# lukashermann/hulc

Hardware: AMD Instinct MI355X
Metric: trajectory-windows/sec (seq_len=32, bs=64/GPU) (higher is better)
Workload: dtype bf16; 1 GPU; HULC training step, vision goal only (use_clip_auxiliary_loss=false), B=64 windows/GPU, seq_len=32, 200x200 static + 84x84 gripper fp32 NCHW frames, fwd+loss+bwd+Adam, dropout 0.1; global_batch=64, seq_len=32, parallelism=dp1

## Files before the change

### hulc_amd/csrc/common.h

```cpp
#pragma once
#include <hip/hip_runtime.h>
#include <stdint.h>

void hulc_set_error(const char* fmt, ...);

#define HIP_CHECK(x)                                                                                     \
    do {                                                                                                 \
        hipError_t e_ = (x);                                                                             \
        if (e_ != hipSuccess) {                                                                          \
            hulc_set_error("%s:%d: %s -> %s", __FILE__, __LINE__, #x, hipGetErrorString(e_));            \
            return 1;                                                                                    \
        }                                                                                                \
    } while (0)

#define DEVI __device__ __forceinline__

#if defined(__HIP_DEVICE_COMPILE__) || defined(__HIPCC__)
__device__ __forceinline__ void lds_dma16(const void* src, unsigned lds_addr) {
    const unsigned a = (unsigned)__builtin_amdgcn_readfirstlane((int)lds_addr);
    asm volatile("s_mov_b32 m0, %1\n\ts_nop 0\n\tglobal_load_lds_dwordx4 %0, off" : : "v"(src), "s"(a) : "memory", "m0");
}
#endif


#ifdef HULC_HALF_F16
#define HULC_NS hulc_f16
#define HULC_HALF_NAME "fp16"
#else
#define HULC_NS hulc_bf16
#define HULC_HALF_NAME "bf16"
#endif

namespace HULC_NS {

typedef uint16_t h16_t;
typedef float f32x4 __attribute__((ext_vector_type(4)));
typedef float f32x2_t __attribute__((ext_vector_type(2)));

#ifdef HULC_HALF_F16
typedef _Float16 h16x8_t __attribute__((ext_vector_type(8)));
typedef _Float16 h16x2_t __attribute__((ext_vector_type(2)));
#define MFMA_16x16x32_H __builtin_amdgcn_mfma_f32_16x16x32_f16
DEVI float h2f(h16_t x) { return (float)*reinterpret_cast<const _Float16*>(&x); }
DEVI h16_t f2h(float f) {
    _Float16 b = (_Float16)f;
    return *reinterpret_cast<h16_t*>(&b);
}
#else
typedef __bf16 h16x8_t __attribute__((ext_vector_type(8)));
typedef __bf16 h16x2_t __attribute__((ext_vector_type(2)));
#define MFMA_16x16x32_H __builtin_amdgcn_mfma_f32_16x16x32_bf16
DEVI float h2f(h16_t x) { return __uint_as_float(((uint32_t)x) << 16); }
DEVI h16_t f2h(float f) {
    __bf16 b = (__bf16)f;
    return *reinterpret_cast<h16_t*>(&b);
}
#endif
DEVI unsigned pack2h(float lo, float hi) {
    h16x2_t b = __builtin_convertvector(f32x2_t{lo, hi}, h16x2_t);
    return *reinterpret_cast<unsigned*>(&b);
}
DEVI float h2f_lo(unsigned w) { return h2f((h16_t)(w & 0xffffu)); }
DEVI float h2f_hi(unsigned w) {
#ifdef HULC_HALF_F16
    return h2f((h16_t)(w >> 16));
#else
    return __uint_as_float(w & 0xffff0000u);
#endif
}
template <typename T> DEVI float to_f(T x);
template <> DEVI float to_f<float>(float x) { return x; }
template <> DEVI float to_f<h16_t>(h16_t x) { return h2f(x); }
template <typename T> DEVI T from_f(float x);
template <> DEVI float from_f<float>(float x) { return x; }
template <> DEVI h16_t from_f<h16_t>(float x) { return f2h(x); }

template <typename T> struct Vec8 { T v[8]; };

template <typename T> DEVI void load8(const T* p, T (&v)[8]);
template <> DEVI void load8<h16_t>(const h16_t* p, h16_t (&v)[8]) {
    if ((((uintptr_t)p) & 15) == 0) {
        uint4 u = *reinterpret_cast<const uint4*>(p);
        *reinterpret_cast<uint4*>(v) = u;
    } else {
#pragma unroll
        for (int i = 0; i < 8; ++i) v[i] = p[i];
    }
}
template <> DEVI void load8<float>(const float* p, float (&v)[8]) {
    if ((((uintptr_t)p) & 15) == 0) {
        float4 a = reinterpret_cast<const float4*>(p)[0];
        float4 b = reinterpret_cast<const float4*>(p)[1];
        v[0] = a.x; v[1] = a.y; v[2] = a.z; v[3] = a.w; v[4] = b.x; v[5] = b.y; v[6] = b.z; v[7] = b.w;
    } else {
#pragma unroll
        for (int i = 0; i < 8; ++i) v[i] = p[i];
    }
}
template <typename T> DEVI void load8_guard(const T* p, int nvalid, T (&v)[8]) {
    if (nvalid >= 8) { load8<T>(p, v); return; }
#pragma unroll
    for (int i = 0; i < 8; ++i) v[i] = (i < nvalid) ? p[i] : from_f<T>(0.f);
}
template <typename T> DEVI void zero8(T (&v)[8]) {
#pragma unroll
    for (int i = 0; i < 8; ++i) v[i] = from_f<T>(0.f);
}

DEVI float wave_sum(float x) {
#pragma unroll
    for (int o = 32; o > 0; o >>= 1) x += __shfl_xor(x, o, 64);
    return x;
}
DEVI float wave_max(float x) {
#pragma unroll
    for (int o = 32; o > 0; o >>= 1) x = fmaxf(x, __shfl_xor(x, o, 64));
    return x;
}

DEVI uint32_t hash_u32(uint64_t seed, uint64_t idx) {
    uint64_t z = seed + (idx + 1) * 0x9E3779B97F4A7C15ull;
    z = (z ^ (z >> 30)) * 0xBF58476D1CE4E5B9ull;
    z = (z ^ (z >> 27)) * 0x94D049BB133111EBull;
    z = z ^ (z >> 31);
    return (uint32_t)(z >> 32);
}
DEVI float hash_uniform(uint64_t seed, uint64_t idx) {
    return ((hash_u32(seed, idx) >> 8) + 0.5f) * (1.0f / 16777216.0f);
}

}
```

### hulc_amd/csrc/tr_fused.h

```cpp
#pragma once
#include "common.h"
#include "conv_wgrad.h"

namespace HULC_NS {

struct TrLayerP {
    const float* xin;
    int ln_in;
    const float *ln_g, *ln_b;
    float* xf_out; h16_t* xt_out; float* st_out;
    const h16_t *Wqkv, *Wo, *W1, *W2;
    const float *bqkv, *bo, *b1, *b2, *n1g, *n1b;
    h16_t* qkv; float* Pat; h16_t* ao; float* y1; float* st1; h16_t* x1t; float* x1f; h16_t* hff; float* y2;
    int B, S;
    float dp;
    unsigned long long seed_att, seed_o, seed_h, seed_y;
    long long* stamps;
};
#ifdef TRF_STAMPS
#define TRF_STAMP(i) do { if (p.stamps && blockIdx.x == 5 && tid == 0) p.stamps[i] = clock64(); } while (0)
#else
#define TRF_STAMP(i) do { } while (0)
#endif

constexpr int TRF_D = 128, TRF_FF = 2048, TRF_NH = 8, TRF_HD = 16, TRF_NQ = 4, TRF_HQ = TRF_FF / TRF_NQ;
constexpr int TRF_XP = TRF_D * 2 + 32;
constexpr int TRF_HP = TRF_HQ * 2 + 32;
constexpr int TRF_QP = 3 * TRF_D * 2 + 16;
constexpr size_t TRF_LDS = 32 * TRF_D * 4 * 2 + 32 * TRF_XP * 3 + 32 * TRF_QP + 32 * TRF_HP;
constexpr size_t TRF_LDS_WIDE = TRF_LDS + 32 * TRF_QP;

template <bool WIDE>
__global__ void __launch_bounds__(512) tr_layer_fwd_kernel(TrLayerP p) {
    extern __shared__ __attribute__((aligned(16))) char smem[];
    typedef __attribute__((address_space(3))) float lds_f32;
    typedef __attribute__((address_space(3))) h16_t lds_h16;
    typedef unsigned int u32x2_t __attribute__((ext_vector_type(2)));
    lds_char* const xf = (lds_char*)smem;
    lds_char* const x1f = xf + 32 * TRF_D * 4;
    lds_char* const xb = x1f + 32 * TRF_D * 4;
    lds_char* const aob = xb + 32 * TRF_XP;
    lds_char* const x1b = aob + 32 * TRF_XP;
    lds_char* const qb = x1b + 32 * TRF_XP;
    lds_char* const hb = qb + (WIDE ? 64 : 32) * TRF_QP;
    const int tid = threadIdx.x, lane = tid & 63, wave = tid >> 6;
    const int li = lane & 15, g = lane >> 4;
    const int hq = blockIdx.x % TRF_NQ;
    const int w = WIDE ? blockIdx.x / (2 * TRF_NQ) : blockIdx.x / TRF_NQ, half = WIDE ? (blockIdx.x / TRF_NQ) & 1 : 0;
    const int SW = p.S;
    const int r0 = half * 32;
    const int S = WIDE ? min(32, SW - r0) : SW;
    const long long row0 = (long long)w * SW + r0;
    const bool lead = hq == 0;
    const bool mt1 = S > 16;
    const float keep = 1.f / (1.f - p.dp);

    TRF_STAMP(0);
    h16x8_t wq[3][4];
#pragma unroll
    for (int nt = 0; nt < 3; ++nt)
#pragma unroll
        for (int ks = 0; ks < 4; ++ks) wq[nt][ks] = *reinterpret_cast<const h16x8_t*>(wfrag_ptr(p.Wqkv, (3 * wave + nt) * 16, TRF_D, 0, lane) + ks * 512);

    f32x4 pbq[3], pb1[4];
#pragma unroll
    for (int nt = 0; nt < 3; ++nt) pbq[nt] = *reinterpret_cast<const f32x4*>(p.bqkv + (3 * wave + nt) * 16 + g * 4);
    const f32x4 pbo = *reinterpret_cast<const f32x4*>(p.bo + wave * 16 + g * 4);
    f32x4 pb2 = f32x4{0.f, 0.f, 0.f, 0.f};
    if (lead) pb2 = *reinterpret_cast<const f32x4*>(p.b2 + wave * 16 + g * 4);
    const float pn1g0 = p.n1g[lane], pn1g1 = p.n1g[lane + 64], pn1b0 = p.n1b[lane], pn1b1 = p.n1b[lane + 64];
    float plg0 = 0.f, plg1 = 0.f, plb0 = 0.f, plb1 = 0.f;
    if (p.ln_in) { plg0 = p.ln_g[lane]; plg1 = p.ln_g[lane + 64]; plb0 = p.ln_b[lane]; plb1 = p.ln_b[lane + 64]; }

    {
#pragma unroll
        for (int rr = 0; rr < 4; ++rr) {
            const int r = wave * 4 + rr;
            float v0 = 0.f, v1 = 0.f;
            if (r < S) {
                const float* xr = p.xin + (row0 + r) * TRF_D;
                v0 = xr[lane]; v1 = xr[lane + 64];
                if (p.ln_in) {
                    const float mean = wave_sum(v0 + v1) * (1.f / TRF_D);
                    const float d0 = v0 - mean, d1 = v1 - mean;
                    const float rstd = rsqrtf(wave_sum(d0 * d0 + d1 * d1) * (1.f / TRF_D) + 1e-5f);
                    v0 = d0 * rstd * plg0 + plb0;
                    v1 = d1 * rstd * plg1 + plb1;
                    if (lead) {
                        p.xf_out[(row0 + r) * TRF_D + lane] = v0; p.xf_out[(row0 + r) * TRF_D + lane + 64] = v1;
                        p.xt_out[(row0 + r) * TRF_D + lane] = f2h(v0); p.xt_out[(row0 + r) * TRF_D + lane + 64] = f2h(v1);
                        if (lane == 0) { p.st_out[2 * (row0 + r)] = mean; p.st_out[2 * (row0 + r) + 1] = rstd; }
                    }
                }
            }
            *(lds_f32*)(xf + (r * TRF_D + lane) * 4) = v0; *(lds_f32*)(xf + (r * TRF_D + lane + 64) * 4) = v1;
            *(lds_h16*)(xb + r * TRF_XP + lane * 2) = f2h(v0); *(lds_h16*)(xb + r * TRF_XP + (lane + 64) * 2) = f2h(v1);
        }
        if (WIDE) {
            const int o0 = 32 - r0, So = min(32, SW - o0);
            const long long orow0 = (long long)w * SW + o0;
#pragma unroll
            for (int rr = 0; rr < 4; ++rr) {
                const int r = wave * 4 + rr;
                float v0 = 0.f, v1 = 0.f;
                if (r < So) {
                    const float* xr = p.xin + (orow0 + r) * TRF_D;
                    v0 = xr[lane]; v1 = xr[lane + 64];
                    if (p.ln_in) {
                        const float mean = wave_sum(v0 + v1) * (1.f / TRF_D);
                        const float d0 = v0 - mean, d1 = v1 - mean;
                        const float rstd = rsqrtf(wave_sum(d0 * d0 + d1 * d1) * (1.f / TRF_D) + 1e-5f);
                        v0 = d0 * rstd * plg0 + plb0;
                        v1 = d1 * rstd * plg1 + plb1;
                    }
                }
                *(lds_h16*)(aob + r * TRF_XP + lane * 2) = f2h(v0); *(lds_h16*)(aob + r * TRF_XP + (lane + 64) * 2) = f2h(v1);
            }
        }
    }
    __syncthreads();
    h16x8_t wo[4], w1[4][4], w2[16];
#pragma unroll
    for (int ks = 0; ks < 4; ++ks) wo[ks] = *reinterpret_cast<const h16x8_t*>(wfrag_ptr(p.Wo, wave * 16, TRF_D, 0, lane) + ks * 512);

    TRF_STAMP(1);
    {
        f32x4 acc[3][2];
#pragma unroll
        for (int nt = 0; nt < 3; ++nt) { acc[nt][0] = f32x4{0.f, 0.f, 0.f, 0.f}; acc[nt][1] = f32x4{0.f, 0.f, 0.f, 0.f}; }
#pragma unroll
        for (int ks = 0; ks < 4; ++ks) {
            const h16x8_t b0 = *(__attribute__((address_space(3))) h16x8_t*)(xb + li * TRF_XP + ks * 64 + g * 16);
            const h16x8_t b1 = *(__attribute__((address_space(3))) h16x8_t*)(xb + (16 + li) * TRF_XP + ks * 64 + g * 16);
#pragma unroll
            for (int nt = 0; nt < 3; ++nt) {
                acc[nt][0] = MFMA_16x16x32_H(wq[nt][ks], b0, acc[nt][0], 0, 0, 0);
                if (mt1) acc[nt][1] = MFMA_16x16x32_H(wq[nt][ks], b1, acc[nt][1], 0, 0, 0);
            }
        }
#pragma unroll
        for (int nt = 0; nt < 3; ++nt) {
            const int n = (3 * wave + nt) * 16 + g * 4;
            const f32x4 bb = pbq[nt];
#pragma unroll
            for (int mt = 0; mt < 2; ++mt) {
                const int m = mt * 16 + li;
                u32x2_t o;
                o[0] = pack2h(acc[nt][mt][0] + bb[0], acc[nt][mt][1] + bb[1]);
                o[1] = pack2h(acc[nt][mt][2] + bb[2], acc[nt][mt][3] + bb[3]);
                *(__attribute__((address_space(3))) u32x2_t*)(qb + (r0 + m) * TRF_QP + n * 2) = o;
                if (lead && m < S) *reinterpret_cast<u32x2_t*>(p.qkv + (row0 + m) * (3 * TRF_D) + n) = o;
            }
        }
        if (WIDE) {
            const int o0 = 32 - r0;
#pragma unroll
            for (int nt = 0; nt < 3; ++nt) { acc[nt][0] = f32x4{0.f, 0.f, 0.f, 0.f}; acc[nt][1] = f32x4{0.f, 0.f, 0.f, 0.f}; }
#pragma unroll
            for (int ks = 0; ks < 4; ++ks) {
                const h16x8_t b0 = *(__attribute__((address_space(3))) h16x8_t*)(aob + li * TRF_XP + ks * 64 + g * 16);
                const h16x8_t b1 = *(__attribute__((address_space(3))) h16x8_t*)(aob + (16 + li) * TRF_XP + ks * 64 + g * 16);
#pragma unroll
                for (int nt = 0; nt < 3; ++nt) {
                    acc[nt][0] = MFMA_16x16x32_H(wq[nt][ks], b0, acc[nt][0], 0, 0, 0);
                    acc[nt][1] = MFMA_16x16x32_H(wq[nt][ks], b1, acc[nt][1], 0, 0, 0);
                }
            }
#pragma unroll
            for (int nt = 0; nt < 3; ++nt) {
                const int n = (3 * wave + nt) * 16 + g * 4;
                const f32x4 bb = pbq[nt];
#pragma unroll
                for (int mt = 0; mt < 2; ++mt) {
                    u32x2_t o;
                    o[0] = pack2h(acc[nt][mt][0] + bb[0], acc[nt][mt][1] + bb[1]);
                    o[1] = pack2h(acc[nt][mt][2] + bb[2], acc[nt][mt][3] + bb[3]);
                    *(__attribute__((address_space(3))) u32x2_t*)(qb + (o0 + mt * 16 + li) * TRF_QP + n * 2) = o;
                }
            }
        }
    }
#pragma unroll
    for (int nt = 0; nt < 4; ++nt) pb1[nt] = *reinterpret_cast<const f32x4*>(p.b1 + hq * TRF_HQ + wave * 64 + nt * 16 + g * 4);
    auto load_w1 = [&]() {
#pragma unroll
        for (int nt = 0; nt < 4; ++nt)
#pragma unroll
            for (int ks = 0; ks < 4; ++ks)
                w1[nt][ks] = *reinterpret_cast<const h16x8_t*>(wfrag_ptr(p.W1, hq * TRF_HQ + wave * 64 + nt * 16, TRF_D, 0, lane) + ks * 512);
    };
    if (!WIDE) load_w1();
    __syncthreads();

    TRF_STAMP(2);
    {
        const int h = wave, i = lane & 31, hf = lane >> 5;
        auto row16 = [&](const lds_char* r, float (&o)[TRF_HD]) {
            const u32x4_t a = *(const lds_u32x4*)r, b = *(const lds_u32x4*)(r + 16);
#pragma unroll
            for (int e = 0; e < 4; ++e) { o[2 * e] = h2f_lo(a[e]); o[2 * e + 1] = h2f_hi(a[e]); o[8 + 2 * e] = h2f_lo(b[e]); o[9 + 2 * e] = h2f_hi(b[e]); }
        };
        constexpr int HJ = WIDE ? 32 : 16;
        if (i < S) {
            float q[TRF_HD];
            row16(qb + (r0 + i) * TRF_QP + h * TRF_HD * 2, q);
#pragma unroll
            for (int d = 0; d < TRF_HD; ++d) q[d] *= 0.25f;
            float sc[HJ];
            float m = -INFINITY;
#pragma unroll
            for (int jj = 0; jj < HJ; ++jj) {
                const int j = hf * HJ + jj;
                float kk[TRF_HD];
                row16(qb + (j < SW ? j : 0) * TRF_QP + (TRF_D + h * TRF_HD) * 2, kk);
                float s = 0.f;
#pragma unroll
                for (int d = 0; d < TRF_HD; ++d) s += q[d] * kk[d];
                sc[jj] = j < SW ? s : -INFINITY;
                m = fmaxf(m, sc[jj]);
            }
            m = fmaxf(m, __shfl_xor(m, 32));
            float den = 0.f;
#pragma unroll
            for (int jj = 0; jj < HJ; ++jj) { sc[jj] = (hf * HJ + jj) < SW ? __expf(sc[jj] - m) : 0.f; den += sc[jj]; }
            den += __shfl_xor(den, 32);
            const float inv = 1.f / den;
            float o[TRF_HD];
#pragma unroll
            for (int d = 0; d < TRF_HD; ++d) o[d] = 0.f;
            const long long pbase = (((long long)w * TRF_NH + h) * SW + r0 + i) * SW;
#pragma unroll
            for (int jj = 0; jj < HJ; ++jj) {
                const int j = hf * HJ + jj;
                if (j < SW) {
                    float pr = sc[jj] * inv;
                    if (lead) p.Pat[pbase + j] = pr;
                    if (p.dp > 0.f) pr = hash_uniform(p.seed_att, (unsigned long long)(pbase + j)) < p.dp ? 0.f : pr * keep;
                    float vv[TRF_HD];
                    row16(qb + j * TRF_QP + (2 * TRF_D + h * TRF_HD) * 2, vv);
#pragma unroll
                    for (int d = 0; d < TRF_HD; ++d) o[d] += pr * vv[d];
                }
            }
#pragma unroll
            for (int d = 0; d < TRF_HD; ++d) o[d] += __shfl_xor(o[d], 32);
            u32x4_t ov;
#pragma unroll
            for (int e = 0; e < 4; ++e) ov[e] = hf ? pack2h(o[8 + 2 * e], o[9 + 2 * e]) : pack2h(o[2 * e], o[2 * e + 1]);
            *(lds_u32x4*)(aob + i * TRF_XP + (h * TRF_HD + hf * 8) * 2) = ov;
            if (lead) *reinterpret_cast<u32x4_t*>(p.ao + (row0 + i) * TRF_D + h * TRF_HD + hf * 8) = ov;
        } else {
            *(lds_u32x4*)(aob + i * TRF_XP + (h * TRF_HD + hf * 8) * 2) = u32x4_t{0u, 0u, 0u, 0u};
        }
    }
    __syncthreads();

    if (WIDE) load_w1();
#pragma unroll
    for (int ks = 0; ks < 16; ++ks) w2[ks] = *reinterpret_cast<const h16x8_t*>(wfrag_ptr(p.W2, wave * 16, TRF_FF, hq * TRF_HQ, lane) + ks * 512);
    TRF_STAMP(3);
    {
        f32x4 acc[2] = {f32x4{0.f, 0.f, 0.f, 0.f}, f32x4{0.f, 0.f, 0.f, 0.f}};
#pragma unroll
        for (int ks = 0; ks < 4; ++ks) {
            const h16x8_t b0 = *(__attribute__((address_space(3))) h16x8_t*)(aob + li * TRF_XP + ks * 64 + g * 16);
            acc[0] = MFMA_16x16x32_H(wo[ks], b0, acc[0], 0, 0, 0);
            if (mt1) {
                const h16x8_t b1 = *(__attribute__((address_space(3))) h16x8_t*)(aob + (16 + li) * TRF_XP + ks * 64 + g * 16);
                acc[1] = MFMA_16x16x32_H(wo[ks], b1, acc[1], 0, 0, 0);
            }
        }
        const int n = wave * 16 + g * 4;
        const f32x4 bb = pbo;
#pragma unroll
        for (int mt = 0; mt < 2; ++mt) {
            const int m = mt * 16 + li;
            lds_char* xr = xf + (m * TRF_D + n) * 4;
            const f32x4 res = *(__attribute__((address_space(3))) f32x4*)xr;
            f32x4 y;
#pragma unroll
            for (int r = 0; r < 4; ++r) {
                float v = acc[mt][r] + bb[r];
                if (p.dp > 0.f) v = hash_uniform(p.seed_o, (unsigned long long)((row0 + m) * TRF_D + n + r)) < p.dp ? 0.f : v * keep;
                y[r] = m < S ? v + res[r] : 0.f;
            }
            *(__attribute__((address_space(3))) f32x4*)xr = y;
            if (lead && m < S) *reinterpret_cast<f32x4*>(p.y1 + (row0 + m) * TRF_D + n) = y;
        }
    }
    __syncthreads();

    TRF_STAMP(4);
    {
#pragma unroll
        for (int rr = 0; rr < 4; ++rr) {
            const int r = wave * 4 + rr;
            float v0 = *(lds_f32*)(xf + (r * TRF_D + lane) * 4), v1 = *(lds_f32*)(xf + (r * TRF_D + lane + 64) * 4);
            float o0 = 0.f, o1 = 0.f;
            if (r < S) {
                const float mean = wave_sum(v0 + v1) * (1.f / TRF_D);
                const float d0 = v0 - mean, d1 = v1 - mean;
                const float rstd = rsqrtf(wave_sum(d0 * d0 + d1 * d1) * (1.f / TRF_D) + 1e-5f);
                o0 = d0 * rstd * pn1g0 + pn1b0;
                o1 = d1 * rstd * pn1g1 + pn1b1;
                if (lead) {
                    p.x1f[(row0 + r) * TRF_D + lane] = o0; p.x1f[(row0 + r) * TRF_D + lane + 64] = o1;
                    p.x1t[(row0 + r) * TRF_D + lane] = f2h(o0); p.x1t[(row0 + r) * TRF_D + lane + 64] = f2h(o1);
                    if (lane == 0) { p.st1[2 * (row0 + r)] = mean; p.st1[2 * (row0 + r) + 1] = rstd; }
                }
            }
            *(lds_f32*)(x1f + (r * TRF_D + lane) * 4) = o0; *(lds_f32*)(x1f + (r * TRF_D + lane + 64) * 4) = o1;
            *(lds_h16*)(x1b + r * TRF_XP + lane * 2) = f2h(o0); *(lds_h16*)(x1b + r * TRF_XP + (lane + 64) * 2) = f2h(o1);
        }
    }
    __syncthreads();

    TRF_STAMP(5);
    {
        f32x4 acc[4][2];
#pragma unroll
        for (int nt = 0; nt < 4; ++nt) { acc[nt][0] = f32x4{0.f, 0.f, 0.f, 0.f}; acc[nt][1] = f32x4{0.f, 0.f, 0.f, 0.f}; }
#pragma unroll
        for (int ks = 0; ks < 4; ++ks) {
            const h16x8_t b0 = *(__attribute__((address_space(3))) h16x8_t*)(x1b + li * TRF_XP + ks * 64 + g * 16);
            const h16x8_t b1 = *(__attribute__((address_space(3))) h16x8_t*)(x1b + (16 + li) * TRF_XP + ks * 64 + g * 16);
#pragma unroll
            for (int nt = 0; nt < 4; ++nt) {
                acc[nt][0] = MFMA_16x16x32_H(w1[nt][ks], b0, acc[nt][0], 0, 0, 0);
                if (mt1) acc[nt][1] = MFMA_16x16x32_H(w1[nt][ks], b1, acc[nt][1], 0, 0, 0);
            }
        }
#pragma unroll
        for (int nt = 0; nt < 4; ++nt) {
            const int nl = wave * 64 + nt * 16 + g * 4, n = hq * TRF_HQ + nl;
            const f32x4 bb = pb1[nt];
#pragma unroll
            for (int mt = 0; mt < 2; ++mt) {
                const int m = mt * 16 + li;
                float v[4];
#pragma unroll
                for (int r = 0; r < 4; ++r) {
                    v[r] = fmaxf(acc[nt][mt][r] + bb[r], 0.f);
                    if (p.dp > 0.f) v[r] = hash_uniform(p.seed_h, (unsigned long long)((row0 + m) * TRF_FF + n + r)) < p.dp ? 0.f : v[r] * keep;
                    if (m >= S) v[r] = 0.f;
                }
                u32x2_t o;
                o[0] = pack2h(v[0], v[1]); o[1] = pack2h(v[2], v[3]);
                *(__attribute__((address_space(3))) u32x2_t*)(hb + m * TRF_HP + nl * 2) = o;
                if (m < S) *reinterpret_cast<u32x2_t*>(p.hff + (row0 + m) * TRF_FF + n) = o;
            }
        }
    }
    __syncthreads();

    TRF_STAMP(6);
    {
        f32x4 acc[2] = {f32x4{0.f, 0.f, 0.f, 0.f}, f32x4{0.f, 0.f, 0.f, 0.f}};
#pragma unroll
        for (int ks = 0; ks < 16; ++ks) {
            const h16x8_t b0 = *(__attribute__((address_space(3))) h16x8_t*)(hb + li * TRF_HP + ks * 64 + g * 16);
            acc[0] = MFMA_16x16x32_H(w2[ks], b0, acc[0], 0, 0, 0);
            if (mt1) {
                const h16x8_t b1 = *(__attribute__((address_space(3))) h16x8_t*)(hb + (16 + li) * TRF_HP + ks * 64 + g * 16);
                acc[1] = MFMA_16x16x32_H(w2[ks], b1, acc[1], 0, 0, 0);
            }
        }
        const int n = wave * 16 + g * 4;
        const f32x4 bb = pb2;
#pragma unroll
        for (int mt = 0; mt < 2; ++mt) {
            const int m = mt * 16 + li;
            if (m >= S) continue;
            const f32x4 res = *(__attribute__((address_space(3))) f32x4*)(x1f + (m * TRF_D + n) * 4);
#pragma unroll
            for (int r = 0; r < 4; ++r) {
                float v = acc[mt][r] + bb[r];
                if (p.dp > 0.f) v = hash_uniform(p.seed_y, (unsigned long long)((row0 + m) * TRF_D + n + r)) < p.dp ? 0.f : v * keep;
                if (lead) v += res[r];
                unsafeAtomicAdd(p.y2 + (row0 + m) * TRF_D + n + r, v);
            }
        }
    }
    TRF_STAMP(7);
}

struct TrFfnBwdP {
    const float* dx; int bcast; float bdiv;
    const float *y2, *st2, *n2g;
    float *dg2, *db2;
    const h16_t *W2t, *W1t;
    const h16_t* hff;
    h16_t *dt_c, *dt_a;
    float* part;
    int B, S; long long N;
    float dp; unsigned long long seed_y;
};
constexpr size_t TRB_LDS = 32 * TRF_D * 4 + 32 * TRF_XP + 32 * TRF_HP + 2 * 8 * 256 * 4;

__global__ void __launch_bounds__(512) tr_ffn_bwd_kernel(TrFfnBwdP p) {
    extern __shared__ __attribute__((aligned(16))) char smem[];
    typedef __attribute__((address_space(3))) float lds_f32;
    typedef __attribute__((address_space(3))) h16_t lds_h16;
    typedef unsigned int u32x2_t __attribute__((ext_vector_type(2)));
    lds_char* const dyf = (lds_char*)smem;
    lds_char* const dcb = dyf + 32 * TRF_D * 4;
    lds_char* const dhb = dcb + 32 * TRF_XP;
    lds_char* const red = dhb + 32 * TRF_HP;
    const int tid = threadIdx.x, lane = tid & 63, wave = tid >> 6;
    const int li = lane & 15, g = lane >> 4;
    const int hq = blockIdx.x % TRF_NQ, nh = (p.S + 31) >> 5, wh = blockIdx.x / TRF_NQ;
    const int w = wh / nh, r0 = (wh % nh) * 32;
    const int S = min(32, p.S - r0);
    const long long row0 = (long long)w * p.S + r0;
    const bool lead = hq == 0;
    const bool mt1 = S > 16;

    h16x8_t w2[4][4];
#pragma unroll
    for (int nt = 0; nt < 4; ++nt)
#pragma unroll
        for (int ks = 0; ks < 4; ++ks)
            w2[nt][ks] = *reinterpret_cast<const h16x8_t*>(wfrag_ptr(p.W2t, hq * TRF_HQ + wave * 64 + nt * 16, TRF_D, 0, lane) + ks * 512);

    {
        const float g0 = p.n2g[lane], g1 = p.n2g[lane + 64];
        float sg0 = 0.f, sg1 = 0.f, sb0 = 0.f, sb1 = 0.f;
#pragma unroll
        for (int rr = 0; rr < 4; ++rr) {
            const int r = wave * 4 + rr;
            float o0 = 0.f, o1 = 0.f, t0 = 0.f, t1 = 0.f;
            if (r < S) {
                const long long row = row0 + r;
                const float mean = p.st2[2 * row], rstd = p.st2[2 * row + 1];
                const float* xr = p.y2 + row * TRF_D;
                const float* dr = p.dx + (p.bcast ? (long long)w : row) * TRF_D;
                const float xh0 = (xr[lane] - mean) * rstd, xh1 = (xr[lane + 64] - mean) * rstd;
                float d0 = dr[lane], d1 = dr[lane + 64];
                if (p.bcast) { d0 /= p.bdiv; d1 /= p.bdiv; }
                sg0 += d0 * xh0; sb0 += d0; sg1 += d1 * xh1; sb1 += d1;
                const float q0 = d0 * g0, q1 = d1 * g1;
                const float m1 = wave_sum(q0 + q1) / TRF_D;
                const float m2 = wave_sum(q0 * xh0 + q1 * xh1) / TRF_D;
                o0 = rstd * (q0 - m1 - xh0 * m2); o1 = rstd * (q1 - m1 - xh1 * m2);
                t0 = o0; t1 = o1;
                if (p.dp > 0.f) {
                    t0 = hash_uniform(p.seed_y, (unsigned long long)(row * TRF_D + lane)) < p.dp ? 0.f : t0 / (1.f - p.dp);
                    t1 = hash_uniform(p.seed_y, (unsigned long long)(row * TRF_D + lane + 64)) < p.dp ? 0.f : t1 / (1.f - p.dp);
                }
                if (lead) { p.dt_c[row * TRF_D + lane] = f2h(t0); p.dt_c[row * TRF_D + lane + 64] = f2h(t1); }
            }
            *(lds_f32*)(dyf + (r * TRF_D + lane) * 4) = o0; *(lds_f32*)(dyf + (r * TRF_D + lane + 64) * 4) = o1;
            *(lds_h16*)(dcb + r * TRF_XP + lane * 2) = f2h(t0); *(lds_h16*)(dcb + r * TRF_XP + (lane + 64) * 2) = f2h(t1);
        }
        if (lead) {
            *(lds_f32*)(red + (wave * 256 + lane) * 4) = sg0; *(lds_f32*)(red + (wave * 256 + 64 + lane) * 4) = sg1;
            *(lds_f32*)(red + (wave * 256 + 128 + lane) * 4) = sb0; *(lds_f32*)(red + (wave * 256 + 192 + lane) * 4) = sb1;
        }
    }
    u32x2_t hm[4][2];
#pragma unroll
    for (int nt = 0; nt < 4; ++nt)
#pragma unroll
        for (int mt = 0; mt < 2; ++mt) {
            const int m = mt * 16 + li;
            hm[nt][mt] = u32x2_t{0u, 0u};
            if (m < S) hm[nt][mt] = *reinterpret_cast<const u32x2_t*>(p.hff + (row0 + m) * TRF_FF + hq * TRF_HQ + wave * 64 + nt * 16 + g * 4);
        }
    h16x8_t w1[16];
#pragma unroll
    for (int ks = 0; ks < 16; ++ks) w1[ks] = *reinterpret_cast<const h16x8_t*>(wfrag_ptr(p.W1t, wave * 16, TRF_FF, hq * TRF_HQ, lane) + ks * 512);
    __syncthreads();
    if (lead && tid < 256) {
        float sum = 0.f;
#pragma unroll
        for (int ww = 0; ww < 8; ++ww) sum += *(lds_f32*)(red + (ww * 256 + tid) * 4);
        unsafeAtomicAdd((tid < 128 ? p.dg2 : p.db2) + (tid & 127), sum);
    }

    {
        const float alpha = p.dp > 0.f ? 1.f / (1.f - p.dp) : 1.f;
        f32x4 acc[4][2];
#pragma unroll
        for (int nt = 0; nt < 4; ++nt) { acc[nt][0] = f32x4{0.f, 0.f, 0.f, 0.f}; acc[nt][1] = f32x4{0.f, 0.f, 0.f, 0.f}; }
#pragma unroll
        for (int ks = 0; ks < 4; ++ks) {
            const h16x8_t b0 = *(__attribute__((address_space(3))) h16x8_t*)(dcb + li * TRF_XP + ks * 64 + g * 16);
            const h16x8_t b1 = *(__attribute__((address_space(3))) h16x8_t*)(dcb + (16 + li) * TRF_XP + ks * 64 + g * 16);
#pragma unroll
            for (int nt = 0; nt < 4; ++nt) {
                acc[nt][0] = MFMA_16x16x32_H(w2[nt][ks], b0, acc[nt][0], 0, 0, 0);
                if (mt1) acc[nt][1] = MFMA_16x16x32_H(w2[nt][ks], b1, acc[nt][1], 0, 0, 0);
            }
        }
#pragma unroll
        for (int nt = 0; nt < 4; ++nt) {
            const int nl = wave * 64 + nt * 16 + g * 4, n = hq * TRF_HQ + nl;
#pragma unroll
            for (int mt = 0; mt < 2; ++mt) {
                const int m = mt * 16 + li;
                float v[4];
#pragma unroll
                for (int r = 0; r < 4; ++r) v[r] = acc[nt][mt][r] * alpha;
                v[0] = h2f_lo(hm[nt][mt][0]) > 0.f ? v[0] : 0.f; v[1] = h2f_hi(hm[nt][mt][0]) > 0.f ? v[1] : 0.f;
                v[2] = h2f_lo(hm[nt][mt][1]) > 0.f ? v[2] : 0.f; v[3] = h2f_hi(hm[nt][mt][1]) > 0.f ? v[3] : 0.f;
                u32x2_t o;
                o[0] = pack2h(v[0], v[1]); o[1] = pack2h(v[2], v[3]);
                if (m >= S) o = u32x2_t{0u, 0u};
                *(__attribute__((address_space(3))) u32x2_t*)(dhb + m * TRF_HP + nl * 2) = o;
                if (m < S) *reinterpret_cast<u32x2_t*>(p.dt_a + (row0 + m) * TRF_FF + n) = o;
            }
        }
    }
    __syncthreads();

    {
        f32x4 acc[2] = {f32x4{0.f, 0.f, 0.f, 0.f}, f32x4{0.f, 0.f, 0.f, 0.f}};
#pragma unroll
        for (int ks = 0; ks < 16; ++ks) {
            const h16x8_t b0 = *(__attribute__((address_space(3))) h16x8_t*)(dhb + li * TRF_HP + ks * 64 + g * 16);
            acc[0] = MFMA_16x16x32_H(w1[ks], b0, acc[0], 0, 0, 0);
            if (mt1) {
                const h16x8_t b1 = *(__attribute__((address_space(3))) h16x8_t*)(dhb + (16 + li) * TRF_HP + ks * 64 + g * 16);
                acc[1] = MFMA_16x16x32_H(w1[ks], b1, acc[1], 0, 0, 0);
            }
        }
        const int n = wave * 16 + g * 4;
        float* const out = p.part + (long long)hq * p.N * TRF_D;
#pragma unroll
        for (int mt = 0; mt < 2; ++mt) {
            const int m = mt * 16 + li;
            if (m >= S) continue;
            f32x4 v = acc[mt];
            if (lead) { const f32x4 res = *(__attribute__((address_space(3))) f32x4*)(dyf + (m * TRF_D + n) * 4); v += res; }
            *reinterpret_cast<f32x4*>(out + (row0 + m) * TRF_D + n) = v;
        }
    }
}
struct TrAttnBwdP {
    const float* parts; long long part_stride; int nparts;
    const float *y1, *st1, *n1g;
    float *dg1, *db1;
    const h16_t *Wot, *Wint;
    const h16_t* qkv; const float* Pat;
    h16_t *b_d, *b_b;
    float *dy_f, *dx;
    int B, S;
    float dp; unsigned long long seed_o, seed_att;
};
constexpr int TRA_HP = 48;
constexpr int TRA_HEADB = 4 * 32 * TRA_HP + 2 * 32 * 33 * 4;
constexpr size_t TRA_LDS = 32 * TRF_XP + 32 * TRF_QP + 8 * 256 * 4 + 8 * TRA_HEADB;

__global__ void __launch_bounds__(512) tr_attn_bwd_kernel(TrAttnBwdP p) {
    extern __shared__ __attribute__((aligned(16))) char smem[];
    typedef __attribute__((address_space(3))) float lds_f32;
    typedef __attribute__((address_space(3))) h16_t lds_h16;
    typedef unsigned int u32x2_t __attribute__((ext_vector_type(2)));
    lds_char* const bdb = (lds_char*)smem;
    lds_char* const dqb = bdb + 32 * TRF_XP;
    lds_char* const red = dqb + 32 * TRF_QP;
    const int tid = threadIdx.x, lane = tid & 63, wave = tid >> 6;
    const int li = lane & 15, g = lane >> 4;
    lds_char* const hb = red + 8 * 256 * 4 + wave * TRA_HEADB;
    lds_char* const qh = hb, * const kh = hb + 32 * TRA_HP, * const vh = hb + 2 * 32 * TRA_HP, * const doh = hb + 3 * 32 * TRA_HP;
    lds_char* const dSb = hb + 4 * 32 * TRA_HP;
    lds_char* const Pdb = dSb + 32 * 33 * 4;
    const int w = blockIdx.x, S = p.S;
    const long long row0 = (long long)w * S;
    const bool mt1 = true;

    h16x8_t wo[4];
#pragma unroll
    for (int ks = 0; ks < 4; ++ks) wo[ks] = *reinterpret_cast<const h16x8_t*>(wfrag_ptr(p.Wot, wave * 16, TRF_D, 0, lane) + ks * 512);

    {
        const float g0 = p.n1g[lane], g1 = p.n1g[lane + 64];
        float sg0 = 0.f, sg1 = 0.f, sb0 = 0.f, sb1 = 0.f;
#pragma unroll
        for (int rr = 0; rr < 4; ++rr) {
            const int r = wave * 4 + rr;
            float t0 = 0.f, t1 = 0.f;
            if (r < S) {
                const long long row = row0 + r;
                const float mean = p.st1[2 * row], rstd = p.st1[2 * row + 1];
                const float* xr = p.y1 + row * TRF_D;
                const float* dr = p.parts + row * TRF_D;
                const float xh0 = (xr[lane] - mean) * rstd, xh1 = (xr[lane + 64] - mean) * rstd;
                float d0 = dr[lane], d1 = dr[lane + 64];
                for (int pp = 1; pp < p.nparts; ++pp) { d0 += dr[pp * p.part_stride + lane]; d1 += dr[pp * p.part_stride + lane + 64]; }
                sg0 += d0 * xh0; sb0 += d0; sg1 += d1 * xh1; sb1 += d1;
                const float q0 = d0 * g0, q1 = d1 * g1;
                const float m1 = wave_sum(q0 + q1) / TRF_D;
                const float m2 = wave_sum(q0 * xh0 + q1 * xh1) / TRF_D;
                const float o0 = rstd * (q0 - m1 - xh0 * m2), o1 = rstd * (q1 - m1 - xh1 * m2);
                p.dy_f[row * TRF_D + lane] = o0; p.dy_f[row * TRF_D + lane + 64] = o1;
                t0 = o0; t1 = o1;
                if (p.dp > 0.f) {
                    t0 = hash_uniform(p.seed_o, (unsigned long long)(row * TRF_D + lane)) < p.dp ? 0.f : t0 / (1.f - p.dp);
                    t1 = hash_uniform(p.seed_o, (unsigned long long)(row * TRF_D + lane + 64)) < p.dp ? 0.f : t1 / (1.f - p.dp);
                }
                p.b_d[row * TRF_D + lane] = f2h(t0); p.b_d[row * TRF_D + lane + 64] = f2h(t1);
            }
            *(lds_h16*)(bdb + r * TRF_XP + lane * 2) = f2h(t0); *(lds_h16*)(bdb + r * TRF_XP + (lane + 64) * 2) = f2h(t1);
        }
        *(lds_f32*)(red + (wave * 256 + lane) * 4) = sg0; *(lds_f32*)(red + (wave * 256 + 64 + lane) * 4) = sg1;
        *(lds_f32*)(red + (wave * 256 + 128 + lane) * 4) = sb0; *(lds_f32*)(red + (wave * 256 + 192 + lane) * 4) = sb1;
    }
    const int ai = lane & 31, hf = lane >> 5;
    if (ai < S) {
        const h16_t* r = p.qkv + (row0 + ai) * 3 * TRF_D + wave * TRF_HD;
        h16_t a0[16], a1[16];
        if (hf == 0) {
            load8<h16_t>(r, *reinterpret_cast<h16_t(*)[8]>(a0)); load8<h16_t>(r + 8, *reinterpret_cast<h16_t(*)[8]>(a0 + 8));
            load8<h16_t>(r + TRF_D, *reinterpret_cast<h16_t(*)[8]>(a1)); load8<h16_t>(r + TRF_D + 8, *reinterpret_cast<h16_t(*)[8]>(a1 + 8));
#pragma unroll
            for (int d = 0; d < 16; ++d) { *(lds_h16*)(qh + ai * TRA_HP + d * 2) = f2h(h2f(a0[d]) * 0.25f); *(lds_h16*)(kh + ai * TRA_HP + d * 2) = a1[d]; }
        } else {
            load8<h16_t>(r + 2 * TRF_D, *reinterpret_cast<h16_t(*)[8]>(a0)); load8<h16_t>(r + 2 * TRF_D + 8, *reinterpret_cast<h16_t(*)[8]>(a0 + 8));
#pragma unroll
            for (int d = 0; d < 16; ++d) *(lds_h16*)(vh + ai * TRA_HP + d * 2) = a0[d];
        }
    }
    h16x8_t wi[12];
#pragma unroll
    for (int ks = 0; ks < 12; ++ks) wi[ks] = *reinterpret_cast<const h16x8_t*>(wfrag_ptr(p.Wint, wave * 16, 3 * TRF_D, 0, lane) + ks * 512);
    __syncthreads();
    if (tid < 256) {
        float sum = 0.f;
#pragma unroll
        for (int ww = 0; ww < 8; ++ww) sum += *(lds_f32*)(red + (ww * 256 + tid) * 4);
        unsafeAtomicAdd((tid < 128 ? p.dg1 : p.db1) + (tid & 127), sum);
    }

    {
        f32x4 acc[2] = {f32x4{0.f, 0.f, 0.f, 0.f}, f32x4{0.f, 0.f, 0.f, 0.f}};
#pragma unroll
        for (int ks = 0; ks < 4; ++ks) {
            const h16x8_t b0 = *(__attribute__((address_space(3))) h16x8_t*)(bdb + li * TRF_XP + ks * 64 + g * 16);
            acc[0] = MFMA_16x16x32_H(wo[ks], b0, acc[0], 0, 0, 0);
            if (mt1) {
                const h16x8_t b1 = *(__attribute__((address_space(3))) h16x8_t*)(bdb + (16 + li) * TRF_XP + ks * 64 + g * 16);
                acc[1] = MFMA_16x16x32_H(wo[ks], b1, acc[1], 0, 0, 0);
            }
        }
#pragma unroll
        for (int mt = 0; mt < 2; ++mt) {
            const int m = mt * 16 + li;
#pragma unroll
            for (int r = 0; r < 4; ++r) *(lds_h16*)(doh + m * TRA_HP + (g * 4 + r) * 2) = f2h(acc[mt][r]);
        }
    }
    __syncthreads();

    auto row16 = [](lds_char* base, int i, float (&x)[16]) {
        const u32x4_t a = *(lds_u32x4*)(base + i * TRA_HP), b = *(lds_u32x4*)(base + i * TRA_HP + 16);
#pragma unroll
        for (int e = 0; e < 4; ++e) { x[2 * e] = h2f_lo(a[e]); x[2 * e + 1] = h2f_hi(a[e]); x[8 + 2 * e] = h2f_lo(b[e]); x[8 + 2 * e + 1] = h2f_hi(b[e]); }
    };
    constexpr int HJ = 16;
    if (ai < S) {
        const float* Pr = p.Pat + (((long long)w * TRF_NH + wave) * S + ai) * S;
        float dot = 0.f;
        float dpv[HJ], pv[HJ];
        float dOi[16];
        row16(doh, ai, dOi);
#pragma unroll
        for (int jj = 0; jj < HJ; ++jj) {
            const int j = hf * HJ + jj;
            dpv[jj] = 0.f; pv[jj] = 0.f;
            if (j < S) {
                float dpj = 0.f, vj[16];
                row16(vh, j, vj);
#pragma unroll
                for (int d = 0; d < 16; ++d) dpj += dOi[d] * vj[d];
                const float pr = Pr[j];
                float keep = 1.f;
                if (p.dp > 0.f) keep = hash_uniform(p.seed_att, (((long long)w * TRF_NH + wave) * S + ai) * S + j) < p.dp ? 0.f : 1.f / (1.f - p.dp);
                *(lds_f32*)(Pdb + (ai * 33 + j) * 4) = pr * keep;
                dpj *= keep;
                dpv[jj] = dpj; pv[jj] = pr;
                dot += dpj * pr;
            }
        }
        dot += __shfl_xor(dot, 32);
#pragma unroll
        for (int jj = 0; jj < HJ; ++jj) if (hf * HJ + jj < S) *(lds_f32*)(dSb + (ai * 33 + hf * HJ + jj) * 4) = pv[jj] * (dpv[jj] - dot);
    }
    __syncthreads();
    if (ai < S) {
        float dq[16], dk[16], dv[16];
#pragma unroll
        for (int d = 0; d < 16; ++d) { dq[d] = 0.f; dk[d] = 0.f; dv[d] = 0.f; }
        for (int jj = 0; jj < HJ; ++jj) {
            const int j = hf * HJ + jj;
            if (j >= S) break;
            const float s_ij = *(lds_f32*)(dSb + (ai * 33 + j) * 4), s_ji = *(lds_f32*)(dSb + (j * 33 + ai) * 4), p_ji = *(lds_f32*)(Pdb + (j * 33 + ai) * 4);
            float kj[16], qj[16], oj[16];
            row16(kh, j, kj); row16(qh, j, qj); row16(doh, j, oj);
#pragma unroll
            for (int d = 0; d < 16; ++d) {
                dq[d] += s_ij * kj[d];
                dk[d] += s_ji * qj[d];
                dv[d] += p_ji * oj[d];
            }
        }
#pragma unroll
        for (int d = 0; d < 16; ++d) { dq[d] += __shfl_xor(dq[d], 32); dk[d] += __shfl_xor(dk[d], 32); dv[d] += __shfl_xor(dv[d], 32); }
        Vec8<h16_t> oq, ok, ov;
#pragma unroll
        for (int d = 0; d < 8; ++d) {
            oq.v[d] = f2h((hf ? dq[8 + d] : dq[d]) * 0.25f); ok.v[d] = f2h(hf ? dk[8 + d] : dk[d]); ov.v[d] = f2h(hf ? dv[8 + d] : dv[d]);
        }
        h16_t* o = p.b_b + (row0 + ai) * 3 * TRF_D + wave * TRF_HD + hf * 8;
        *reinterpret_cast<Vec8<h16_t>*>(o) = oq; *reinterpret_cast<Vec8<h16_t>*>(o + TRF_D) = ok; *reinterpret_cast<Vec8<h16_t>*>(o + 2 * TRF_D) = ov;
        lds_char* lo = dqb + ai * TRF_QP + (wave * TRF_HD + hf * 8) * 2;
        *(lds_u32x4*)(lo) = __builtin_bit_cast(u32x4_t, oq);
        *(lds_u32x4*)(lo + TRF_D * 2) = __builtin_bit_cast(u32x4_t, ok);
        *(lds_u32x4*)(lo + 2 * TRF_D * 2) = __builtin_bit_cast(u32x4_t, ov);
    }
    __syncthreads();

    {
        f32x4 acc[2] = {f32x4{0.f, 0.f, 0.f, 0.f}, f32x4{0.f, 0.f, 0.f, 0.f}};
#pragma unroll
        for (int ks = 0; ks < 12; ++ks) {
            const h16x8_t b0 = *(__attribute__((address_space(3))) h16x8_t*)(dqb + li * TRF_QP + ks * 64 + g * 16);
            acc[0] = MFMA_16x16x32_H(wi[ks], b0, acc[0], 0, 0, 0);
            if (mt1) {
                const h16x8_t b1 = *(__attribute__((address_space(3))) h16x8_t*)(dqb + (16 + li) * TRF_QP + ks * 64 + g * 16);
                acc[1] = MFMA_16x16x32_H(wi[ks], b1, acc[1], 0, 0, 0);
            }
        }
        const int n = wave * 16 + g * 4;
#pragma unroll
        for (int mt = 0; mt < 2; ++mt) {
            const int m = mt * 16 + li;
            if (m >= S) continue;
            const f32x4 res = *reinterpret_cast<const f32x4*>(p.dy_f + (row0 + m) * TRF_D + n);
            *reinterpret_cast<f32x4*>(p.dx + (row0 + m) * TRF_D + n) = acc[mt] + res;
        }
    }
}
static inline void launch_tr_attn_bwd(hipStream_t st, const TrAttnBwdP& p) {
    static bool attr_set = false;
    if (!attr_set) { hipFuncSetAttribute((const void*)tr_attn_bwd_kernel, hipFuncAttributeMaxDynamicSharedMemorySize, (int)TRA_LDS); attr_set = true; }
    hipLaunchKernelGGL(tr_attn_bwd_kernel, dim3(p.B), dim3(512), TRA_LDS, st, p);
}

static inline void launch_tr_ffn_bwd(hipStream_t st, const TrFfnBwdP& p) {
    static bool attr_set = false;
    if (!attr_set) { hipFuncSetAttribute((const void*)tr_ffn_bwd_kernel, hipFuncAttributeMaxDynamicSharedMemorySize, (int)TRB_LDS); attr_set = true; }
    hipLaunchKernelGGL(tr_ffn_bwd_kernel, dim3(p.B * ((p.S + 31) / 32) * TRF_NQ), dim3(512), TRB_LDS, st, p);
}

static inline void launch_tr_layer_fwd(hipStream_t st, const TrLayerP& p) {
    static bool attr_set = false;
    if (!attr_set) {
        hipFuncSetAttribute((const void*)tr_layer_fwd_kernel<false>, hipFuncAttributeMaxDynamicSharedMemorySize, (int)TRF_LDS);
        hipFuncSetAttribute((const void*)tr_layer_fwd_kernel<true>, hipFuncAttributeMaxDynamicSharedMemorySize, (int)TRF_LDS_WIDE);
        attr_set = true;
    }
    if (p.S > 32) hipLaunchKernelGGL(tr_layer_fwd_kernel<true>, dim3(p.B * 2 * TRF_NQ), dim3(512), TRF_LDS_WIDE, st, p);
    else hipLaunchKernelGGL(tr_layer_fwd_kernel<false>, dim3(p.B * TRF_NQ), dim3(512), TRF_LDS, st, p);
}

}
```

Measured before the change: 21920 windows/s.

## Compute attention backward dP and dQ/dK/dV with MFMA instead of scalar loops

Replaces the per-thread scalar dot-product loops in the fused transformer attention backward with matrix instructions. dP = dO·V^T uses a 32x32x16 half MFMA, and dQ, dK and dV use fp32 16x16x4 MFMAs reading dS and P from LDS. Padding rows of Q/K/V in LDS are now zeroed so the fixed-size MFMA tiles read clean data. The aim is to cut ALU and LDS-read cost in the backward attention stage. The risk is changed accumulation order and precision for dP, which now takes bf16 inputs via MFMA.

```diff
diff --git a/hulc_amd/csrc/common.h b/hulc_amd/csrc/common.h
--- a/hulc_amd/csrc/common.h
+++ b/hulc_amd/csrc/common.h
@@ -56,6 +56,7 @@
     return *reinterpret_cast<h16_t*>(&b);
 }
 #endif
+#define MFMA_16x16x4_F32 __builtin_amdgcn_mfma_f32_16x16x4f32
 DEVI unsigned pack2h(float lo, float hi) {
     h16x2_t b = __builtin_convertvector(f32x2_t{lo, hi}, h16x2_t);
     return *reinterpret_cast<unsigned*>(&b);
diff --git a/hulc_amd/csrc/tr_fused.h b/hulc_amd/csrc/tr_fused.h
--- a/hulc_amd/csrc/tr_fused.h
+++ b/hulc_amd/csrc/tr_fused.h
@@ -1,6 +1,7 @@
 #pragma once
 #include "common.h"
 #include "conv_wgrad.h"
+#include "conv_reg.h"
 
 namespace HULC_NS {
 
@@ -620,6 +621,10 @@
 #pragma unroll
             for (int d = 0; d < 16; ++d) *(lds_h16*)(vh + ai * TRA_HP + d * 2) = a0[d];
         }
+    } else {
+        const u32x4_t z = u32x4_t{0u, 0u, 0u, 0u};
+        if (hf == 0) { *(lds_u32x4*)(qh + ai * TRA_HP) = z; *(lds_u32x4*)(qh + ai * TRA_HP + 16) = z; *(lds_u32x4*)(kh + ai * TRA_HP) = z; *(lds_u32x4*)(kh + ai * TRA_HP + 16) = z; }
+        else { *(lds_u32x4*)(vh + ai * TRA_HP) = z; *(lds_u32x4*)(vh + ai * TRA_HP + 16) = z; }
     }
     h16x8_t wi[12];
 #pragma unroll
@@ -652,71 +657,77 @@
     }
     __syncthreads();
 
-    auto row16 = [](lds_char* base, int i, float (&x)[16]) {
-        const u32x4_t a = *(lds_u32x4*)(base + i * TRA_HP), b = *(lds_u32x4*)(base + i * TRA_HP + 16);
-#pragma unroll
-        for (int e = 0; e < 4; ++e) { x[2 * e] = h2f_lo(a[e]); x[2 * e + 1] = h2f_hi(a[e]); x[8 + 2 * e] = h2f_lo(b[e]); x[8 + 2 * e + 1] = h2f_hi(b[e]); }
-    };
-    constexpr int HJ = 16;
-    if (ai < S) {
-        const float* Pr = p.Pat + (((long long)w * TRF_NH + wave) * S + ai) * S;
+    {
+        const bool rowok = ai < S;
+        const long long pbase = (((long long)w * TRF_NH + wave) * S + ai) * S;
+        const float* Pr = p.Pat + pbase;
+        f32x16 dpt;
+#pragma unroll
+        for (int r = 0; r < 16; ++r) dpt[r] = 0.f;
+        {
+            const h16x8_t av = *(__attribute__((address_space(3))) h16x8_t*)(vh + ai * TRA_HP + hf * 16);
+            const h16x8_t bo = *(__attribute__((address_space(3))) h16x8_t*)(doh + ai * TRA_HP + hf * 16);
+            dpt = MFMA_32x32x16_H(av, bo, dpt, 0, 0, 0);
+        }
+        float pv[16];
         float dot = 0.f;
-        float dpv[HJ], pv[HJ];
-        float dOi[16];
-        row16(doh, ai, dOi);
-#pragma unroll
-        for (int jj = 0; jj < HJ; ++jj) {
-            const int j = hf * HJ + jj;
-            dpv[jj] = 0.f; pv[jj] = 0.f;
-            if (j < S) {
-                float dpj = 0.f, vj[16];
-                row16(vh, j, vj);
-#pragma unroll
-                for (int d = 0; d < 16; ++d) dpj += dOi[d] * vj[d];
-                const float pr = Pr[j];
+#pragma unroll
+        for (int r = 0; r < 16; ++r) {
+            const int j = 8 * (r >> 2) + 4 * hf + (r & 3);
+            float pr = 0.f, dpj = 0.f, pd = 0.f;
+            if (rowok && j < S) {
+                pr = Pr[j];
                 float keep = 1.f;
-                if (p.dp > 0.f) keep = hash_uniform(p.seed_att, (((long long)w * TRF_NH + wave) * S + ai) * S + j) < p.dp ? 0.f : 1.f / (1.f - p.dp);
-                *(lds_f32*)(Pdb + (ai * 33 + j) * 4) = pr * keep;
-                dpj *= keep;
-                dpv[jj] = dpj; pv[jj] = pr;
-                dot += dpj * pr;
-            }
+                if (p.dp > 0.f) keep = hash_uniform(p.seed_att, pbase + j) < p.dp ? 0.f : 1.f / (1.f - p.dp);
+                pd = pr * keep;
+                dpj = dpt[r] * keep;
+            }
+            *(lds_f32*)(Pdb + (ai * 33 + j) * 4) = pd;
+            dpt[r] = dpj; pv[r] = pr;
+            dot += dpj * pr;
         }
         dot += __shfl_xor(dot, 32);
 #pragma unroll
-        for (int jj = 0; jj < HJ; ++jj) if (hf * HJ + jj < S) *(lds_f32*)(dSb + (ai * 33 + hf * HJ + jj) * 4) = pv[jj] * (dpv[jj] - dot);
-    }
-    __syncthreads();
-    if (ai < S) {
-        float dq[16], dk[16], dv[16];
-#pragma unroll
-        for (int d = 0; d < 16; ++d) { dq[d] = 0.f; dk[d] = 0.f; dv[d] = 0.f; }
-        for (int jj = 0; jj < HJ; ++jj) {
-            const int j = hf * HJ + jj;
-            if (j >= S) break;
-            const float s_ij = *(lds_f32*)(dSb + (ai * 33 + j) * 4), s_ji = *(lds_f32*)(dSb + (j * 33 + ai) * 4), p_ji = *(lds_f32*)(Pdb + (j * 33 + ai) * 4);
-            float kj[16], qj[16], oj[16];
-            row16(kh, j, kj); row16(qh, j, qj); row16(doh, j, oj);
-#pragma unroll
-            for (int d = 0; d < 16; ++d) {
-                dq[d] += s_ij * kj[d];
-                dk[d] += s_ji * qj[d];
-                dv[d] += p_ji * oj[d];
-            }
-        }
-#pragma unroll
-        for (int d = 0; d < 16; ++d) { dq[d] += __shfl_xor(dq[d], 32); dk[d] += __shfl_xor(dk[d], 32); dv[d] += __shfl_xor(dv[d], 32); }
-        Vec8<h16_t> oq, ok, ov;
-#pragma unroll
-        for (int d = 0; d < 8; ++d) {
-            oq.v[d] = f2h((hf ? dq[8 + d] : dq[d]) * 0.25f); ok.v[d] = f2h(hf ? dk[8 + d] : dk[d]); ov.v[d] = f2h(hf ? dv[8 + d] : dv[d]);
-        }
-        h16_t* o = p.b_b + (row0 + ai) * 3 * TRF_D + wave * TRF_HD + hf * 8;
-        *reinterpret_cast<Vec8<h16_t>*>(o) = oq; *reinterpret_cast<Vec8<h16_t>*>(o + TRF_D) = ok; *reinterpret_cast<Vec8<h16_t>*>(o + 2 * TRF_D) = ov;
-        lds_char* lo = dqb + ai * TRF_QP + (wave * TRF_HD + hf * 8) * 2;
-        *(lds_u32x4*)(lo) = __builtin_bit_cast(u32x4_t, oq);
-        *(lds_u32x4*)(lo + TRF_D * 2) = __builtin_bit_cast(u32x4_t, ok);
-        *(lds_u32x4*)(lo + 2 * TRF_D * 2) = __builtin_bit_cast(u32x4_t, ov);
+        for (int r = 0; r < 16; ++r) {
+            const int j = 8 * (r >> 2) + 4 * hf + (r & 3);
+            *(lds_f32*)(dSb + (ai * 33 + j) * 4) = (rowok && j < S) ? pv[r] * (dpt[r] - dot) : 0.f;
+        }
+    }
+    __syncthreads();
+    {
+        f32x4 aq[2], ak[2], av[2];
+#pragma unroll
+        for (int nt = 0; nt < 2; ++nt) { aq[nt] = f32x4{0.f, 0.f, 0.f, 0.f}; ak[nt] = f32x4{0.f, 0.f, 0.f, 0.f}; av[nt] = f32x4{0.f, 0.f, 0.f, 0.f}; }
+#pragma unroll
+        for (int ks = 0; ks < 8; ++ks) {
+            const int kk = ks * 4 + g;
+            const float k_a = h2f(*(lds_h16*)(kh + kk * TRA_HP + li * 2));
+            const float q_a = h2f(*(lds_h16*)(qh + kk * TRA_HP + li * 2));
+            const float o_a = h2f(*(lds_h16*)(doh + kk * TRA_HP + li * 2));
+#pragma unroll
+            for (int nt = 0; nt < 2; ++nt) {
+                const int t = nt * 16 + li;
+                aq[nt] = MFMA_16x16x4_F32(k_a, *(lds_f32*)(dSb + (t * 33 + kk) * 4), aq[nt], 0, 0, 0);
+                ak[nt] = MFMA_16x16x4_F32(q_a, *(lds_f32*)(dSb + (kk * 33 + t) * 4), ak[nt], 0, 0, 0);
+                av[nt] = MFMA_16x16x4_F32(o_a, *(lds_f32*)(Pdb + (kk * 33 + t) * 4), av[nt], 0, 0, 0);
+            }
+        }
+#pragma unroll
+        for (int nt = 0; nt < 2; ++nt) {
+            const int t = nt * 16 + li;
+            u32x2_t oq, ok, ov;
+            oq[0] = pack2h(aq[nt][0] * 0.25f, aq[nt][1] * 0.25f); oq[1] = pack2h(aq[nt][2] * 0.25f, aq[nt][3] * 0.25f);
+            ok[0] = pack2h(ak[nt][0], ak[nt][1]); ok[1] = pack2h(ak[nt][2], ak[nt][3]);
+            ov[0] = pack2h(av[nt][0], av[nt][1]); ov[1] = pack2h(av[nt][2], av[nt][3]);
+            if (t < S) {
+                h16_t* o = p.b_b + (row0 + t) * 3 * TRF_D + wave * TRF_HD + g * 4;
+                *reinterpret_cast<u32x2_t*>(o) = oq; *reinterpret_cast<u32x2_t*>(o + TRF_D) = ok; *reinterpret_cast<u32x2_t*>(o + 2 * TRF_D) = ov;
+            }
+            lds_char* lo = dqb + t * TRF_QP + (wave * TRF_HD + g * 4) * 2;
+            *(__attribute__((address_space(3))) u32x2_t*)(lo) = oq;
+            *(__attribute__((address_space(3))) u32x2_t*)(lo + TRF_D * 2) = ok;
+            *(__attribute__((address_space(3))) u32x2_t*)(lo + 2 * TRF_D * 2) = ov;
+        }
     }
     __syncthreads();
 
```

After: 22040 windows/s, median of 6. No clear change (+0.5%).
